# vqdang/hover_net

Measured on AMD Instinct MI355X. Metric: tiles/sec (270x270, batch 32) end-to-end incl. watershed, higher is better.
Workload: dtype fp32

## Files before the change

### hover_net_amd/csrc/hvn_api.hip

```cpp
#include <hip/hip_runtime.h>
#include <stdio.h>
#include <string.h>

#include <vector>

#include "../../include/hvn.h"
#include "hvn_kernels.h"

static thread_local char g_err[512] = "";

static int fail(int code, const char *fmt, const char *a = "", long b = 0)
{
    snprintf(g_err, sizeof(g_err), fmt, a, b);
    return code;
}

extern "C" {

int hvn_version(void) { return 104; }

#ifndef HVN_BUILD_ID
#define HVN_BUILD_ID "unstamped"
#endif
static const char hvn_build_tag[] = "hvn-build-id:" HVN_BUILD_ID;
// ... 141 lines not shown
        a.xsn = op->x.sn; a.xsy = op->x.sy; a.xsx = op->x.sx; a.K1 = op->x.c;
        a.x2 = (const float *)op->x2.base;
        a.x2sn = op->x2.sn; a.x2sy = op->x2.sy; a.x2sx = op->x2.sx;
        a.K1b = a.x2 ? op->x2.c : 0;
        a.stride2 = op->_rsv > 0 ? op->_rsv : 1;
        a.w1 = op->w;
        a.res = (const float *)op->res.base;
        a.rsn = op->res.sn; a.rsy = op->res.sy; a.rsx = op->res.sx;
        a.y = (float *)op->y.base;
        a.ysn = op->y.sn; a.ysy = op->y.sy; a.ysx = op->y.sx; a.C = op->cout;
        a.post_s = op->post_scale; a.post_b = op->post_shift;
        a.pre_s = op->pre_scale; a.pre_b = op->pre_shift;
        a.w2 = op->w2; a.bias2 = op->bias2; a.relu2 = 1;
        a.y2 = (float *)op->y2.base;
        a.y2sn = op->y2.sn; a.y2sy = op->y2.sy; a.y2sx = op->y2.sx; a.N2 = op->cout2;
        a.N = batch; a.Ho = op->y.h; a.Wo = op->y.w;
        a.M = (long)batch * a.Ho * a.Wo;
        a.bm = op->tile_n == 64 ? 64 : 128;
        const bool cx3 = op->act_dtype == 2 || op->act_dtype == 3;
        const bool cbf = op->act_dtype == 1;
        if (op->act_dtype != 0 && !cx3 && !cbf) return fail(HVN_E_ARG, "chain: act_dtype 0 (fp32), 1 (bf16) or 2 | 3 (fp32 with bf16x3 products)%s", "");
        if (cbf) {
            if (!a.x || !a.w1 || !a.y || !a.w2 || !a.y2) return fail(HVN_E_ARG, "chain: null pointer%s", "");
            if (op->kh != 1 || op->kw != 1 || op->stride != 1 || op->pad_t || op->pad_l || op->relu || op->bias)
                return fail(HVN_E_ARG, "chain: the first conv is a plain 1x1 (no bias / relu of its own)%s", "");
            if (!hvn_chain_bf16_supported(a.K1, a.K1b, a.C, a.N2) || op->y.c != a.C || op->y2.c != a.N2)
                return fail(HVN_E_ARG, "chain (bf16): needs input channels in slabs of 64 (64 or 128 in all), cout %% 256 == 0, cout2 in {64, 128} (cout2 = %s%ld)", "", a.N2);
            if (op->x.h != a.Ho || op->x.w != a.Wo || op->y2.h != a.Ho || op->y2.w != a.Wo ||
                (a.x2 && ((long)(a.Ho - 1) * a.stride2 >= op->x2.h || (long)(a.Wo - 1) * a.stride2 >= op->x2.w)))
                return fail(HVN_E_ARG, "chain: views do not cover the output grid%s", "");
            if (a.res && (a.rsn != a.ysn || a.rsy != a.ysy || a.rsx != a.ysx || op->res.c != a.C))
                return fail(HVN_E_ARG, "chain: the residual view must have the output's strides%s", "");
            if (!aligned16(a.x) || !aligned16(a.w1) || !aligned16(a.w2) || !aligned16(a.y) || !aligned16(a.y2) || (a.res && !aligned16(a.res)) ||
                (a.x2 && !aligned16(a.x2)) || ((a.xsn | a.xsy | a.xsx | a.ysn | a.ysy | a.ysx | a.y2sn | a.y2sy | a.y2sx | a.x2sn | a.x2sy | a.x2sx) & 7))
                return fail(HVN_E_ARG, "chain (bf16): views / weights not 16-byte aligned%s", "");
            if ((!a.pre_s != !a.pre_b) || (!a.post_s != !a.post_b) || (a.pre_s && (!aligned16(a.pre_s) || !aligned16(a.pre_b))) ||
                (a.post_s && (!aligned16(a.post_s) || !aligned16(a.post_b))) || (a.bias2 && !aligned16(a.bias2)))
                return fail(HVN_E_ARG, "chain: per-channel vectors must be 16-byte aligned and come in pairs%s", "");
            if (g_prof) prof_mark(s);
            const int rcb = hvn_launch_conv_chain_bf16(a, s);
            if (g_prof) prof_mark(s);
            if (rcb) return fail(rcb == -1 ? HVN_E_ARG : HVN_E_LAUNCH, "chain (bf16): launch failed (cout2=%s%ld)", "", a.N2);
            return 0;
        }
        if (!a.x || !a.w1 || !a.y || !a.w2 || !a.y2) return fail(HVN_E_ARG, "chain: null pointer%s", "");
        if (op->kh != 1 || op->kw != 1 || op->stride != 1 || op->pad_t || op->pad_l || op->relu || op->bias)
            return fail(HVN_E_ARG, "chain: the first conv is a plain 1x1 (no bias / relu of its own)%s", "");
        if (!hvn_chain_supported(a.C, a.N2) || op->y.c != a.C || op->y2.c != a.N2 || a.K1 % 32 || a.K1b % 32 || a.K1 + a.K1b < 64)
            return fail(HVN_E_ARG, "chain: needs cout %% 64 == 0, cout2 in {64, 128}, input channels in slabs of 32 (>= 64) (cout2 = %s%ld)", "", a.N2);
        if (op->x.h != a.Ho || op->x.w != a.Wo || op->y2.h != a.Ho || op->y2.w != a.Wo ||
            (a.x2 && ((long)(a.Ho - 1) * a.stride2 >= op->x2.h || (long)(a.Wo - 1) * a.stride2 >= op->x2.w)))
            return fail(HVN_E_ARG, "chain: views do not cover the output grid%s", "");
        if (a.res && (a.rsn != a.ysn || a.rsy != a.ysy || a.rsx != a.ysx || op->res.c != a.C))
            return fail(HVN_E_ARG, "chain: the residual view must have the output's strides%s", "");
        if (!aligned16(a.x) || !aligned16(a.w1) || !aligned16(a.w2) || !aligned16(a.y) || !aligned16(a.y2) || (a.res && !aligned16(a.res)) ||
            (a.x2 && !aligned16(a.x2)) || ((a.xsn | a.xsy | a.xsx | a.ysn | a.ysy | a.ysx | a.y2sn | a.y2sy | a.y2sx | a.x2sn | a.x2sy | a.x2sx) & 3))
            return fail(HVN_E_ARG, "chain: views / weights not 16-byte aligned%s", "");
        if ((!a.pre_s != !a.pre_b) || (!a.post_s != !a.post_b) || (a.pre_s && (!aligned16(a.pre_s) || !aligned16(a.pre_b))) ||
            (a.post_s && (!aligned16(a.post_s) || !aligned16(a.post_b))) || (a.bias2 && !aligned16(a.bias2)))
            return fail(HVN_E_ARG, "chain: per-channel vectors must be 16-byte aligned and come in pairs%s", "");
        if (g_prof) prof_mark(s);
        int rc;
        if (cx3 && op->tile_n == 1152)
            rc = hvn_launch_conv_chain_x3r(a, op->act_dtype == 3 ? 6 : 9, s);
        else
            rc = cx3 ? hvn_launch_conv_chain_x3(a, op->act_dtype == 3 ? 6 : 9, s) : hvn_launch_conv_chain(a, s);
        if (g_prof) prof_mark(s);
        if (rc) return fail(rc == -1 ? HVN_E_ARG : HVN_E_LAUNCH, "chain: launch failed (cout2=%s%ld)", "", a.N2);
        return 0;
    }
    case HVN_OP_WINO_IN:
    case HVN_OP_WINO_OUT: {
        WinoArgs a;
        const bool in = op->kind == HVN_OP_WINO_IN;
        a.x = (const float *)op->x.base;
        a.xsn = op->x.sn; a.xsy = op->x.sy; a.xsx = op->x.sx;
        a.y = (float *)op->y.base;
        a.ysn = op->y.sn; a.ysy = op->y.sy; a.ysx = op->y.sx;
        a.mat = op->w; a.bias = op->bias;
        a.N = batch; a.H = in ? op->x.h : op->y.h; a.W = in ? op->x.w : op->y.w; a.C = in ? op->x.c : op->y.c;
        a.ty = op->kh; a.tx = op->kw; a.pad = op->pad_t; a.relu = op->relu;
        a.accum = (!in && op->res.base != nullptr) ? 1 : 0;
        a.lo = nullptr; a.lsn = a.lsy = a.lsx = 0;
        if (in && op->res.base) {
            a.lo = (const float *)op->res.base;
            a.lsn = op->res.sn; a.lsy = op->res.sy; a.lsx = op->res.sx;
            if (op->res.h * 2 != op->x.h || op->res.w * 2 != op->x.w || op->res.c != op->x.c || !aligned16(a.lo) || ((a.lsn | a.lsy | a.lsx) & 3))
                return fail(HVN_E_ARG, "wino_in: the half-resolution input must be x.h/2 x x.w/2 x x.c and 16-byte aligned%s", "");
        }
        if (a.accum && op->res.base != op->y.base) return fail(HVN_E_ARG, "wino_out: res must alias y (accumulate in place)%s", "");
        const int n2 = in ? op->y.h : op->x.h;
        if (op->stride > 1 && op->_rsv > 1) {
            a.m = op->stride; a.r = op->_rsv;
        } else {
            a.m = n2 == 36 ? 2 : n2 == 64 ? 4 : n2 == 100 ? 6 : 0; a.r = 5;
        }
        if (!a.m || (a.m + a.r - 1) * (a.m + a.r - 1) != n2 || !((a.m == 2 && a.r == 5) || ((a.m == 4 || a.m == 6) && (a.r == 5 || a.r == 3))))
            return fail(HVN_E_ARG, "winograd transform: %s%ld transform positions do not match F(2,5) / F(4,5) / F(4,3) / F(6,3) / F(6,5)", "", (long)n2);
        if (!a.x || !a.y || !a.mat || a.ty <= 0 || a.tx <= 0 || (a.C & 3)) return fail(HVN_E_ARG, "winograd transform: bad descriptor%s", "");
        if (!aligned16(a.x) || !aligned16(a.y) || ((a.xsn | a.xsy | a.xsx | a.ysn | a.ysy | a.ysx) & 3))
            return fail(HVN_E_ARG, "winograd transform: views not 16-byte aligned%s", "");
        if (in && (op->y.w != a.ty * a.tx || op->y.c != a.C)) return fail(HVN_E_ARG, "wino_in: V must be [n*n][tiles][c]%s", "");
        if (!in && (op->x.w != a.ty * a.tx || op->y.h > a.m * a.ty || op->y.h <= a.m * (a.ty - 1) || op->y.w > a.m * a.tx ||
                    op->y.w <= a.m * (a.tx - 1) || op->x.c != a.C))
            return fail(HVN_E_ARG, "wino_out: M must be [n*n][tiles][cout] and the tiles must cover y%s", "");
        if (g_prof) prof_mark(s);
        int rc = in ? hvn_launch_wino_in(a, s) : hvn_launch_wino_out(a, s);
        if (g_prof) prof_mark(s);
        return rc;
    }
    case HVN_OP_UPADD: {
        UpAddArgs a;
        a.lo = (const float *)op->x.base;
        a.lsn = op->x.sn; a.lsy = op->x.sy; a.lsx = op->x.sx;
        a.skip = (const float *)op->res.base;
        a.ssn = op->res.sn; a.ssy = op->res.sy; a.ssx = op->res.sx;
        a.y = (float *)op->y.base;
        a.ysn = op->y.sn; a.ysy = op->y.sy; a.ysx = op->y.sx;
        a.N = batch; a.H = op->y.h; a.W = op->y.w; a.C = op->y.c; a.bf16 = op->act_dtype == 1;
        if (a.bf16 && ((a.lsx | a.lsy | a.lsn | a.ssx | a.ssy | a.ssn | a.ysx | a.ysy | a.ysn) & 7))
            return fail(HVN_E_ARG, "upadd(bf16): strides must be multiples of 8 elements%s", "");
        if (!a.lo || !a.skip || !a.y) return fail(HVN_E_ARG, "upadd: null pointer%s", "");
        if (op->x.h * 2 != a.H || op->x.w * 2 != a.W || op->res.h != a.H || op->res.w != a.W || op->x.c != a.C || op->res.c != a.C)
            return fail(HVN_E_ARG, "upadd: shape mismatch%s", "");
        if (!aligned16(a.lo) || !aligned16(a.skip) || !aligned16(a.y) || ((a.lsx | a.lsy | a.lsn | a.ssx | a.ssy | a.ssn | a.ysx | a.ysy | a.ysn) & 3))
            return fail(HVN_E_ARG, "upadd: views not 16-byte aligned%s", "");
        return hvn_launch_upadd(a, s);
    }
    case HVN_OP_HEAD: {
        HeadArgs a;
        a.x = (const float *)op->x.base;
        a.xsn = op->x.sn; a.xsy = op->x.sy; a.xsx = op->x.sx;
        a.w = op->w; a.bias = op->bias;
        a.y = (float *)op->y.base;
        a.N = batch; a.H = op->x.h; a.W = op->x.w; a.Cout = op->cout; a.in_bf16 = op->act_dtype == 1;
        if (a.in_bf16 && ((a.xsx | a.xsy | a.xsn) & 7)) return fail(HVN_E_ARG, "head(bf16): strides must be multiples of 8 elements%s", "");
        if (op->x.c != 64 || !a.w || !a.bias || !a.x || !a.y) return fail(HVN_E_ARG, "head: expects 64 input channels, weights and bias%s", "");
        if (!aligned16(a.x) || ((a.xsx | a.xsy | a.xsn) & 3)) return fail(HVN_E_ARG, "head: input view not 16-byte aligned%s", "");
        return hvn_launch_head(a, s);
    }
    case HVN_OP_PREDMAP: {
        PredMapArgs a;
        a.np = (const float *)op->x.base;
        a.hv = (const float *)op->res.base;
        a.tp = op->w;
        a.y = (float *)op->y.base;
        a.N = batch; a.H = op->y.h; a.W = op->y.w; a.nr_types = op->cout;
        if (!a.np || !a.hv || !a.y || (a.nr_types > 0 && !a.tp)) return fail(HVN_E_ARG, "predmap: null pointer%s", "");
        if (a.nr_types > 0 && !aligned16(a.y)) return fail(HVN_E_ARG, "predmap: output not 16-byte aligned%s", "");
        return hvn_launch_predmap(a, s);
    }
    default:
        return fail(HVN_E_ARG, "unknown op kind %s%ld", "", op->kind);
    }
}

}
int hvn_internal_run_one(const hvn_op *op, int batch, hipStream_t s) { return run_one(op, batch, s); }
extern "C" {

int hvn_run_op(const hvn_op *op, int batch, void *stream)
{
    if (!op || batch <= 0) return fail(HVN_E_ARG, "run_op: bad arguments%s", "");
    int rc = run_one(op, batch, (hipStream_t)stream);
    if (rc == -2) return fail(HVN_E_LAUNCH, "launch failed: %s", hipGetErrorString(hipGetLastError()));
    return rc;
// ... 102 lines not shown
```

### hover_net_amd/csrc/hvn_kernels.h

```cpp
#pragma once
#include <hip/hip_runtime.h>
#include <stdint.h>

#include <atomic>

static inline int hvn_max_lds_once(const void *kern, int bytes, std::atomic<unsigned long long> &done)
{
    int dev = 0;
    if (hipGetDevice(&dev) != hipSuccess) return -2;
    const unsigned long long bit = 1ull << (dev & 63);
    if (done.load(std::memory_order_acquire) & bit) return 0;
    if (hipFuncSetAttribute(kern, hipFuncAttributeMaxDynamicSharedMemorySize, bytes) != hipSuccess) return -2;
    done.fetch_or(bit, std::memory_order_release);
    return 0;
}

struct ConvArgs {
    const float *x;
    long xsn, xsy, xsx;
    int H, W, Cin;
    const float *w;
    const float *bias, *pre_s, *pre_b, *post_s, *post_b;
    const float *res;
    long rsn, rsy, rsx;
// ... 56 lines not shown
int hvn_launch_conv_chain_x3r(const ChainArgs &a, int terms, hipStream_t stream);
int hvn_launch_conv_bf16(const ConvArgs &a, int tile_n, hipStream_t stream);
int hvn_launch_conv_bf16g(const ConvArgs &a, int bm, hipStream_t stream);
int hvn_launch_conv_x3(const ConvArgs &a, int tile_n, int terms, hipStream_t stream);
int hvn_launch_conv_x3g(const ConvArgs &a, int bm, int terms, hipStream_t stream);
int hvn_conv_x3g_supported(const ConvArgs &a, int bm);
int hvn_launch_split_x3(const float *src, uint16_t *dst, long granules, hipStream_t stream);

struct Conv0Args {
    const void *img;
    long isn, isy, isx, isc;
    int is_f32;
    int H, W;
    const float *w;
    const float *bias;
    float *y;
    long ysn, ysy, ysx;
    int N, Ho, Wo, pad;
    int relu;
    int out_bf16;
};
int hvn_launch_conv0(const Conv0Args &a, hipStream_t stream);

struct UpAddArgs {
    const float *lo;
    long lsn, lsy, lsx;
    const float *skip;
    long ssn, ssy, ssx;
    float *y;
    long ysn, ysy, ysx;
    int N, H, W, C;
    int bf16;
};
int hvn_launch_upadd(const UpAddArgs &a, hipStream_t stream);

struct HeadArgs {
    const float *x;
    long xsn, xsy, xsx;
    const float *w;
    const float *bias;
    float *y;
    int N, H, W, Cout;
    int in_bf16;
};
int hvn_launch_head(const HeadArgs &a, hipStream_t stream);

int hvn_launch_extract_patches(const uint8_t *img, int H, int W, const int32_t *coords, int P, int win, int pad_t, int pad_l, uint8_t *out,
                               hipStream_t stream);

int hvn_launch_resize_window(const uint8_t *src, int src_h, int src_w, int64_t src_pitch, int src_y0, int src_x0, int full_h, int full_w,
                             const int32_t *xofs, const int16_t *xcoef, const int32_t *yofs, const int16_t *ycoef, int taps, uint8_t *dst,
                             int dst_h, int dst_w, hipStream_t stream);

size_t hvn_tissue_workspace_bytes(int h, int w);
int hvn_launch_tissue_gray_hist(const uint8_t *rgb, int h, int w, uint8_t *gray, uint32_t *hist256, hipStream_t stream);
int hvn_launch_tissue_mask(const uint8_t *gray, int h, int w, int threshold, int min_obj, int max_hole, int radius, uint8_t *mask,
                           uint8_t *tap_objects, uint8_t *tap_holes, void *workspace, hipStream_t stream);

int hvn_launch_viz_strip(const uint8_t *img, int n, int ih, int iw, const float *pred, int c, const int32_t *np_map, const float *hv_map,
                         const int32_t *tp_map, int h, int w, int nr_types, const int32_t *sel, int n_sel, const uint8_t *lut, uint8_t *out,
                         int n_blocks, hipStream_t stream);

struct PredMapArgs {
    const float *tp, *np, *hv;
    float *y;
    int N, H, W, nr_types;
};
int hvn_launch_predmap(const PredMapArgs &a, hipStream_t stream);

struct WinoArgs {
    const float *x;
    long xsn, xsy, xsx;
    float *y;
    long ysn, ysy, ysx;
    const float *mat;
    const float *bias;
    int N, H, W, C;
    int ty, tx, pad, relu;
    int m;
    int r;
    int accum;
    const float *lo;
    long lsn, lsy, lsx;
};
int hvn_launch_wino_in(const WinoArgs &a, hipStream_t stream);
int hvn_launch_wino_out(const WinoArgs &a, hipStream_t stream);

struct PackArgs {
    const float *src;
    float *dst;
    int cout, cin_g, groups, taps;
    int mode;
    int lead_pad;
    const float *gmat;
};
int hvn_launch_pack_w(const PackArgs &a, hipStream_t stream);
int hvn_launch_pack_w_multi(const PackArgs *tbl, const int *first_block, int n, long blocks, hipStream_t stream);

struct WgradArgs {
    const float *x;
    long xsn, xsy, xsx;
    int H, W, Cin;
    const float *dy;
    long dsn, dsy, dsx;
    int Ho, Wo, Cout;
    float *dw;
    int N, KH, KW, stride, pad_t, pad_l, groups, Cin_g;
    int tiles_m, tiles_n;
    unsigned rows_per_split;
    int nbatch;
    long xb, db, wb;
    int want_wgs;
    float *part;
    long part_stride, part_cap;
};
int hvn_launch_wgrad(const WgradArgs &a, hipStream_t stream);
long hvn_wgrad_split(const WgradArgs &a, long tiles, unsigned *rows_per_split);
long hvn_wgrad_part_floats(const WgradArgs &a, int x3);
int hvn_launch_reduce_parts(float *dst, const float *part, long elems, long nparts, long stride, hipStream_t stream);
int hvn_wgrad_x3_supported(const WgradArgs &a);
int hvn_launch_wgrad_x3(WgradArgs a, int terms, hipStream_t stream);
int hvn_launch_wino_dy(const struct WinoArgs &a, hipStream_t stream);
int hvn_launch_wino_dw(const float *du, float *dg, const float *gmat, int cout, int cin, hipStream_t stream);

#define HVN_BN_MAX_PARTS 256
struct BnArgs {
    const float *z;
    long zsn, zsy, zsx;
    const float *a;
    float *a_out;
    long asn, asy, asx;
    const float *da;
    long gsn, gsy, gsx;
    float *dz;
    long dsn, dsy, dsx;
    double *ws;
    float *save;
    float *coef;
    const float *gamma, *beta;
    float *dgamma, *dbeta, *running_mean, *running_var;
    int N, H, W, C, lq, nparts;
    float eps, momentum;
    int dz_store;
};
int hvn_launch_bn_forward(BnArgs a, hipStream_t stream);
int hvn_launch_bn_backward(BnArgs a, hipStream_t stream);

struct UpAddBwdArgs {
    const float *dy;
    long ysn, ysy, ysx;
    float *dlo;
    long lsn, lsy, lsx;
    float *dskip;
    long ssn, ssy, ssx;
    int N, H, W, C;
};
int hvn_launch_upadd_bwd(const UpAddBwdArgs &a, hipStream_t stream);

struct HeadBwdArgs {
    const float *x;
    long xsn, xsy, xsx;
    float *dx;
    long dsn, dsy, dsx;
    const float *dl;
    const float *w;
    float *dw, *db;
// ... 59 lines not shown
```

### hover_net_amd/csrc/hvn_net_ops.hip

```cpp
#include <hip/hip_runtime.h>
#include <stdlib.h>
#include <stdint.h>

#include "hvn_conv_common.h"

#define C0_T 16
#define C0_P (C0_T + 6)
template <typename T>
__global__ __launch_bounds__(256) void hvn_conv0(const Conv0Args p)
{
    __shared__ float patch[C0_P][C0_P * 3 + 2];
    const int tid = threadIdx.x;
    const int n = blockIdx.z;
    const int oy0 = blockIdx.y * C0_T, ox0 = blockIdx.x * C0_T;
    const T *img = (const T *)p.img + (long)n * p.isn;
    for (int i = tid; i < C0_P * C0_P * 3; i += 256) {
        const int py = i / (C0_P * 3), pr = i - py * (C0_P * 3);
        const int px = pr / 3, ch = pr - px * 3;
        const int iy = oy0 + py - p.pad, ix = ox0 + px - p.pad;
        float v = 0.f;
        if ((unsigned)iy < (unsigned)p.H && (unsigned)ix < (unsigned)p.W) v = (float)img[(long)iy * p.isy + (long)ix * p.isx + (long)ch * p.isc];
        patch[py][pr] = v;
    }
    __syncthreads();
// ... 247 lines not shown
        *(float4 *)(p.y + i * 4) = make_float4((float)best, prob, h, v);
    } else {
        float *y = p.y + i * 3;
        y[0] = prob;
        y[1] = h;
        y[2] = v;
    }
}

int hvn_launch_predmap(const PredMapArgs &a, hipStream_t stream)
{
    const long total = (long)a.N * a.H * a.W;
    hipLaunchKernelGGL(hvn_predmap, dim3((unsigned)((total + 255) / 256)), dim3(256), 0, stream, a, total);
    return hipGetLastError() == hipSuccess ? 0 : -2;
}

#ifndef HVN_WINO_XCD
#define HVN_WINO_XCD 1
#endif
template <int VW> struct WVec;
template <> struct WVec<4> { typedef float T __attribute__((ext_vector_type(4))); };
template <> struct WVec<2> { typedef float T __attribute__((ext_vector_type(2))); };
template <> struct WVec<1> { typedef float T __attribute__((ext_vector_type(1))); };

template <int MO, int R, int VW>
__global__ __launch_bounds__(256) void hvn_wino_in(const WinoArgs p, long total)
{
    constexpr int NW = MO + R - 1;
    typedef typename WVec<VW>::T VT;
    unsigned bid = blockIdx.x;
#if HVN_WINO_XCD
    {
        const unsigned per = gridDim.x >> 3;
        if (bid < per * 8) bid = (bid & 7) * per + (bid >> 3);
    }
#endif
    const long i = (long)bid * 256 + threadIdx.x;
    if (i >= total) return;
    const int cvn = p.C / VW;
    const int cv = (int)(i % cvn);
    long t = i / cvn;
    const int T1 = p.ty * p.tx;
    const int tile = (int)(t % T1);
    const int n = (int)(t / T1);
    const int tyi = tile / p.tx, txi = tile - tyi * p.tx;
    const int y0 = MO * tyi - p.pad, x0 = MO * txi - p.pad;
    float bt[NW * NW];
#pragma unroll
    for (int k = 0; k < NW * NW; ++k) bt[k] = p.mat[k];
    const float *src = p.x + (long)n * p.xsn + cv * VW;
    const float *lo = p.lo ? p.lo + (long)n * p.lsn + cv * VW : nullptr;
    VT tmp[NW][NW];
#pragma unroll
    for (int j = 0; j < NW; ++j) {
        VT d[NW];
#pragma unroll
        for (int r = 0; r < NW; ++r) {
            const int yy = y0 + r, xx = x0 + j;
            const bool in = (unsigned)yy < (unsigned)p.H && (unsigned)xx < (unsigned)p.W;
            VT v = in ? *(const VT *)(src + (long)yy * p.xsy + (long)xx * p.xsx) : (VT)(0.f);
            if (lo && in) v = *(const VT *)(lo + (long)(yy >> 1) * p.lsy + (long)(xx >> 1) * p.lsx) + v;
            d[r] = v;
        }
#pragma unroll
        for (int a = 0; a < NW; ++a) {
            VT s = (VT)(0.f);
#pragma unroll
            for (int r = 0; r < NW; ++r) s = __builtin_elementwise_fma((VT)(bt[a * NW + r]), d[r], s);
            tmp[a][j] = s;
        }
    }
    float *dst = p.y + (long)n * p.ysn + (long)tile * p.ysx + cv * VW;
#pragma unroll
    for (int a = 0; a < NW; ++a)
#pragma unroll
        for (int b = 0; b < NW; ++b) {
            VT s = (VT)(0.f);
#pragma unroll
            for (int j = 0; j < NW; ++j) s = __builtin_elementwise_fma((VT)(bt[b * NW + j]), tmp[a][j], s);
            *(VT *)(dst + (long)(a * NW + b) * p.ysy) = s;
        }
}

int hvn_launch_wino_in(const WinoArgs &a, hipStream_t stream)
{
    if (a.m == 2 && a.r == 5) {
        const long total = (long)a.N * a.ty * a.tx * (a.C / 4);
        hipLaunchKernelGGL((hvn_wino_in<2, 5, 4>), dim3((unsigned)((total + 255) / 256)), dim3(256), 0, stream, a, total);
    } else if (a.m == 4 && a.r == 3) {
        const long total = (long)a.N * a.ty * a.tx * (a.C / 4);
        hipLaunchKernelGGL((hvn_wino_in<4, 3, 4>), dim3((unsigned)((total + 255) / 256)), dim3(256), 0, stream, a, total);
    } else if (a.m == 4 && a.r == 5) {
        const long total = (long)a.N * a.ty * a.tx * (a.C / 2);
        hipLaunchKernelGGL((hvn_wino_in<4, 5, 2>), dim3((unsigned)((total + 255) / 256)), dim3(256), 0, stream, a, total);
    } else if (a.m == 6 && a.r == 3) {
        const long total = (long)a.N * a.ty * a.tx * (a.C / 2);
        hipLaunchKernelGGL((hvn_wino_in<6, 3, 2>), dim3((unsigned)((total + 255) / 256)), dim3(256), 0, stream, a, total);
    } else if (a.m == 6 && a.r == 5) {
        const long total = (long)a.N * a.ty * a.tx * a.C;
        hipLaunchKernelGGL((hvn_wino_in<6, 5, 1>), dim3((unsigned)((total + 255) / 256)), dim3(256), 0, stream, a, total);
    } else
        return -1;
    return hipGetLastError() == hipSuccess ? 0 : -2;
}

template <int MO, int R, int VW>
__global__ __launch_bounds__(256) void hvn_wino_out(const WinoArgs p, long total)
{
    constexpr int NW = MO + R - 1;
    typedef typename WVec<VW>::T VT;
    const long i = (long)blockIdx.x * 256 + threadIdx.x;
    if (i >= total) return;
    const int c4n = p.C / VW;
    const int c4 = (int)(i % c4n);
    long t = i / c4n;
    const int T1 = p.ty * p.tx;
    const int tile = (int)(t % T1);
    const int n = (int)(t / T1);
    const int tyi = tile / p.tx, txi = tile - tyi * p.tx;
    float at[MO * NW];
#pragma unroll
    for (int k = 0; k < MO * NW; ++k) at[k] = p.mat[k];
    const float *src = p.x + (long)n * p.xsn + (long)tile * p.xsx + c4 * VW;
    VT tmp[MO][NW];
#pragma unroll
    for (int b = 0; b < NW; ++b) {
        VT m[NW];
#pragma unroll
        for (int a = 0; a < NW; ++a) m[a] = *(const VT *)(src + (long)(a * NW + b) * p.xsy);
#pragma unroll
        for (int q = 0; q < MO; ++q) {
            VT s = (VT)(0.f);
#pragma unroll
            for (int a = 0; a < NW; ++a) s = __builtin_elementwise_fma((VT)(at[q * NW + a]), m[a], s);
            tmp[q][b] = s;
        }
    }
    VT bias = (VT)(0.f);
    if (p.bias) bias = *(const VT *)(p.bias + c4 * VW);
    const float lo = p.relu ? 0.f : -__builtin_inff();
    float *dst = p.y + (long)n * p.ysn + c4 * VW;
#pragma unroll
    for (int q = 0; q < MO; ++q)
#pragma unroll
        for (int r = 0; r < MO; ++r) {
            VT s = bias;
#pragma unroll
            for (int b = 0; b < NW; ++b) s = __builtin_elementwise_fma((VT)(at[r * NW + b]), tmp[q][b], s);
            s = __builtin_elementwise_max(s, (VT)(lo));
            const int oy = MO * tyi + q, ox = MO * txi + r;
            if (oy < p.H && ox < p.W) {
                VT *d = (VT *)(dst + (long)oy * p.ysy + (long)ox * p.ysx);
                *d = p.accum ? *d + s : s;
            }
        }
}

int hvn_launch_wino_out(const WinoArgs &a, hipStream_t stream)
{
    if (a.m == 2 && a.r == 5) {
        const long total = (long)a.N * a.ty * a.tx * (a.C / 4);
        hipLaunchKernelGGL((hvn_wino_out<2, 5, 4>), dim3((unsigned)((total + 255) / 256)), dim3(256), 0, stream, a, total);
    } else if (a.m == 4 && a.r == 3) {
        const long total = (long)a.N * a.ty * a.tx * (a.C / 4);
        hipLaunchKernelGGL((hvn_wino_out<4, 3, 4>), dim3((unsigned)((total + 255) / 256)), dim3(256), 0, stream, a, total);
    } else if (a.m == 4 && a.r == 5) {
        const long total = (long)a.N * a.ty * a.tx * (a.C / 2);
        hipLaunchKernelGGL((hvn_wino_out<4, 5, 2>), dim3((unsigned)((total + 255) / 256)), dim3(256), 0, stream, a, total);
// ... 46 lines not shown
```

### hover_net_amd/engine.py

```python
import ctypes

import numpy as np
import torch

from . import lib as L
from . import plan as PL
from . import tune as T
from .tune import X3G_128, X3G_256, X3R


def _view_struct(v, base_ptr, sn, itemsize=4):
    b = v.buf
    sx = b.c
    sy = b.w * b.c
    s = L.hvn_view()
    s.base = base_ptr + (v.y0 * sy + v.x0 * sx + v.c0) * itemsize
    s.sn, s.sy, s.sx = sn, sy, sx
    s.h, s.w, s.c, s.sc = v.h, v.w, v.c, 1
    return s


_STREAM_POOL = {}


# ... 5 lines not shown


def to_bf16_bits(a):
    u = np.ascontiguousarray(a, np.float32).view(np.uint32)
    return ((u + (((u >> 16) & 1) + 0x7FFF)) >> 16).astype(np.uint16)


def repack_conv_bf16(w32):
    cp, s32, taps, _ = w32.shape
    if s32 % 2:
        w32 = np.concatenate([w32, np.zeros((cp, 1, taps, 32), np.float32)], 1)
        s32 += 1
    w = w32.reshape(cp, s32 // 2, 2, taps, 32).transpose(0, 1, 3, 2, 4).reshape(cp, s32 // 2, taps, 64)
    return to_bf16_bits(w)


def split_bf16x3(w32):
    w = np.ascontiguousarray(w32, np.float32)

    def bf(a):
        bits = to_bf16_bits(a)
        return bits, (bits.astype(np.uint32) << 16).view(np.float32)

    h, hf = bf(w)
    r = w - hf
    m, mf = bf(r)
    l, _ = bf(r - mf)
    return h, m, l


def pack_conv_x3(w32):
    lead = w32.shape[:-3]
    kt = w32.shape[-3] * w32.shape[-2]
    planes = split_bf16x3(w32.reshape(lead + (kt, 32)))
    return np.stack(planes, axis=-2)


def pack_conv_x3_device(w32, device):
    w = torch.from_numpy(np.ascontiguousarray(w32, np.float32).reshape(-1, 32)).to(device)
    h = w.to(torch.bfloat16)
    r = w - h.float()
    m = r.to(torch.bfloat16)
    l = (r - m.float()).to(torch.bfloat16)
    return torch.stack((h, m, l), dim=1).view(torch.int16).reshape(-1)


class Engine:
    def __init__(self, plan, max_batch=32, device="cuda", n_split=None, dtype="fp32", n_lanes=None):
        L.require_gpu()
        assert dtype in ("fp32", "bf16")
        self.dtype = dtype
        self.isz = 4 if dtype == "fp32" else 2
        if dtype == "bf16" and any(op.kind in (PL.OP_WINO_IN, PL.OP_WINO_OUT) for op in plan.ops):
            raise ValueError("the bf16 path runs direct convolutions: build the plan with winograd=0")
        self.plan = plan
        self.max_batch = int(max_batch)
        self.device = torch.device(device)
        import os
        dflt = ("2", "2") if dtype == "fp32" else ("1", "0")
        self.n_split = int(os.environ.get("HVN_SPLIT", dflt[0])) if n_split is None else int(n_split)
        self.n_lane_streams = int(os.environ.get("HVN_LANES", dflt[1])) if n_lanes is None else int(n_lanes)
        self.split_decoder = os.environ.get("HVN_SPLIT_DECODER", "0") != "0"
        self._streams = None
        self._stream_off = 0
        self._upload_params()
        self.arena = torch.empty((self.max_batch, plan.arena_per_sample), dtype=torch.float32 if dtype == "fp32" else torch.int16,
                                 device=self.device)
        self.logits = {br: torch.empty((self.max_batch, b.c, b.h, b.w), dtype=torch.float32, device=self.device)
                       for br, b in plan.logits.items()}
        self.pred_map = None
        if plan.pred_map is not None:
            pm = plan.pred_map
            self.pred_map = torch.empty((self.max_batch, pm.h, pm.w, pm.c), dtype=torch.float32, device=self.device)
        self.ops = (L.hvn_op * len(plan.ops))()
        self._bind()
        self._sub_ops = {}
        tile_file = T.knob("HVN_TILE_FILE")
        if tile_file and dtype == "fp32":
            import json
            tiles = json.load(open(tile_file))
            if len(tiles) != len(self.ops):
                raise ValueError("HVN_TILE_FILE holds %d entries for a plan of %d ops" % (len(tiles), len(self.ops)))
            for o, tn in zip(self.ops, tiles):
                if tn in T.candidates(o):
                    o.tile_n = tn
        elif T.tile_select() == "auto" and not (dtype == "fp32" and T.knob("HVN_FORCE_TILE_N")):
            self.autotune_tiles()
        if T.tile_select() == "auto" and T.knob("HVN_STREAM_SELECT") != "0":
            self.autotune_streams()

    def _upload_params(self):
        arrays, offs, total = [], {}, 0

        def put(key, a):
            nonlocal total
            if a is None:
                return
            a = np.ascontiguousarray(a, np.float32).ravel()
            offs[key] = total
            arrays.append((total, a))
            total += (a.size + 63) // 64 * 64

        w16, off16, tot16 = [], {}, 0
        for i, op in enumerate(self.plan.ops):
            if self.dtype == "bf16" and op.kind in (PL.OP_CONV, PL.OP_CHAIN):
                wb = repack_conv_bf16(op.w).ravel()
                off16[i] = tot16
                w16.append((tot16, wb))
                tot16 += (wb.size + 127) // 128 * 128
                if op.kind == PL.OP_CHAIN:
                    wb2 = repack_conv_bf16(op.extra["w2"]).ravel()
                    off16[(i, "w2")] = tot16
                    w16.append((tot16, wb2))
                    tot16 += (wb2.size + 127) // 128 * 128
            elif self.dtype == "fp32" and op.kind in (PL.OP_CONV, PL.OP_CHAIN) and op.extra.get("x3"):
                off16[i] = tot16
                w16.append((tot16, op.w, True))
                tot16 += (3 * op.w.size + 127) // 128 * 128
                if op.kind == PL.OP_CHAIN:
                    off16[(i, "w2")] = tot16
                    w16.append((tot16, op.extra["w2"], True))
                    tot16 += (3 * op.extra["w2"].size + 127) // 128 * 128
            else:
                put((i, "w"), op.w)
            put((i, "bias"), op.bias)
            if not (op.kind == PL.OP_CHAIN and (self.dtype == "bf16" or op.extra.get("x3"))):
                put((i, "w2"), op.extra.get("w2"))
            put((i, "bias2"), op.extra.get("bias2"))
            if op.pre is not None:
                put((i, "pre_s"), op.pre[0])
                put((i, "pre_b"), op.pre[1])
            if op.post is not None:
                put((i, "post_s"), op.post[0])
                put((i, "post_b"), op.post[1])
        host = np.zeros(max(total, 64), np.float32)
        for off, a in arrays:
            host[off:off + a.size] = a
        self.params = torch.from_numpy(host).to(self.device)
        self._poff = offs
        self._poff16 = off16
        self.params16 = None
        if tot16:
            if any(len(e) == 3 for e in w16):
                self.params16 = torch.zeros(tot16, dtype=torch.int16, device=self.device)
                for off, w32, _ in w16:
                    pl = pack_conv_x3_device(w32, self.device)
                    self.params16[off:off + pl.numel()] = pl
            else:
                h16 = np.zeros(tot16, np.uint16)
                for off, a in w16:
                    h16[off:off + a.size] = a
                self.params16 = torch.from_numpy(h16.view(np.int16)).to(self.device)

    def _pptr(self, i, name):
        off = self._poff.get((i, name))
        return None if off is None else self.params.data_ptr() + 4 * off

    def _bind(self):
        P = self.plan
        abase = self.arena.data_ptr()
        sn = P.arena_per_sample
        for i, op in enumerate(P.ops):
            o = self.ops[i]
            o.act_dtype = 1 if self.dtype == "bf16" else 0
            o.kind, o.kh, o.kw, o.stride = op.kind, op.kh, op.kw, op.stride
            o.pad_t, o.pad_l, o.relu, o.cout, o.tile_n, o.x_dtype = op.pad_t, op.pad_l, op.relu, op.cout, op.tile_n, 0
            if op.kind == PL.OP_CONV and self.dtype == "fp32":
                o.tile_n = T.pick_tile_n(op, self.max_batch)
            o.groups = int(op.extra.get("groups", 1))
            o._rsv = int(op.extra.get("stride2", 1))
            o.nbatch = int(op.extra.get("nbatch", 1))
            for bi, bs in enumerate(op.extra.get("batch_strides", (0, 0, 0))):
                o.batch_stride[bi] = int(bs)
            if op.kind in (PL.OP_WINO_IN, PL.OP_WINO_OUT):
                o.kh, o.kw = op.extra["tiles"]
                o.stride, o._rsv = op.extra["m"], op.extra.get("r", 5)
            if op.kind == PL.OP_PREDMAP:
                o.x.base = self.logits["np"].data_ptr()
                o.res.base = self.logits["hv"].data_ptr()
                o.w = self.logits["tp"].data_ptr() if "tp" in self.logits else None
                o.cout = P.nr_types or 0
                o.y.base = self.pred_map.data_ptr()
                o.y.h, o.y.w, o.y.c = P.pred_map.h, P.pred_map.w, P.pred_map.c
                continue
            if op.kind == PL.OP_CHAIN:
                o.cout2 = int(op.extra["cout2"])
                o.w2, o.bias2 = self._pptr(i, "w2"), self._pptr(i, "bias2")
                if self.dtype == "bf16":
                    o.w2 = self.params16.data_ptr() + 2 * self._poff16[(i, "w2")]
                elif op.extra.get("x3"):
                    o.w2 = self.params16.data_ptr() + 2 * self._poff16[(i, "w2")]
                    o.act_dtype = 2 if int(op.extra["x3"]) == 9 else 3
                    o.tile_n = 128
            for fld, v in (("x", op.x), ("res", op.res), ("y", op.y), ("x2", op.extra.get("x2")), ("y2", op.extra.get("y2"))):
                if v is None:
                    continue
                if v.buf.offset >= 0:
                    setattr(o, fld, _view_struct(v, abase + self.isz * v.buf.offset, sn, self.isz))
            if op.kind == PL.OP_CONV0:
                o.x.h, o.x.w, o.x.c = op.x.h, op.x.w, 3
            if op.kind == PL.OP_HEAD:
                br = op.y.buf.name.split(".")[1]
                o.y.base = self.logits[br].data_ptr()
                o.y.h, o.y.w, o.y.c = op.y.h, op.y.w, op.y.c
            o.w = self._pptr(i, "w") if i not in self._poff16 else self.params16.data_ptr() + 2 * self._poff16[i]
            if i in self._poff16 and self.dtype == "bf16":
                o.groups = 1
            if self.dtype == "fp32" and op.kind == PL.OP_CONV and op.extra.get("x3"):
                o.act_dtype = 2 if int(op.extra["x3"]) == 9 else 3
                if o.nbatch > 1:
                    o.batch_stride[1] = int(op.w.shape[-4]) * int(op.w.shape[-3]) * int(op.w.shape[-2]) * 96
            o.bias = self._pptr(i, "bias")
            o.pre_scale, o.pre_shift = self._pptr(i, "pre_s"), self._pptr(i, "pre_b")
            o.post_scale, o.post_shift = self._pptr(i, "post_s"), self._pptr(i, "post_b")

    def autotune_streams(self):
        split = self.n_split if (self.n_split > 1 and self.max_batch >= 2 * self.n_split) else 1
        need = (split - 1) + split * self.n_lane_streams
        if need == 0 or self.plan.ops[0].kind != PL.OP_CONV0 or not getattr(self.plan, "geo", None):
            return
        g = int(self.plan.geo.get("inp", 0))
        if g <= 0:
            return
        imgs = torch.zeros((self.max_batch, g, g, 3), dtype=torch.uint8, device=self.device)

        def measure(off):
            self._stream_off, self._streams = off, None
            return T.time_launch(lambda: self.run(imgs), runs=2)

        key = (str(self.device), "streams", split, self.n_lane_streams, self.dtype)
        self._stream_off, self._streams = T.choose(T.CACHE, key, (0, 1, 2, 3), measure, margin=1.0)[0], None

    def autotune_tiles(self):
        run_op = L.lib().hvn_run_op
        stream = L.stream_ptr(self.device)
        osz = ctypes.sizeof(L.hvn_op)
        base = ctypes.addressof(self.ops)
        lanes = getattr(self.plan, "lanes", None)
        enc_end = lanes[0][2] if (lanes and lanes[0][0] == "main" and len(lanes) > 1) else 0
        split = self.n_split if (self.n_split > 1 and self.max_batch >= 2 * self.n_split) else 1
        sub_n = -(-self.max_batch // split) if T.knob("HVN_TUNE_SUB") != "0" else self.max_batch
        for i, o in enumerate(self.ops):
            cands = T.candidates(o)
            if not cands:
                continue
            nb = sub_n if (i < enc_end or self.split_decoder) else self.max_batch
            family = "infer-bf16" if o.act_dtype == 1 else "infer-conv" if o.kind == PL.OP_CONV else "infer-chain-x3" if o.act_dtype else "infer-chain"

            def measure(tn):
                o.tile_n = tn
                return T.time_launch(lambda: L.check(run_op(base + i * osz, nb, stream), "hvn_run_op (autotune)"))

            o.tile_n = T.pick(T.CACHE, T.launch_key(self.device, family, o, nb), cands, measure, forced=T.forced_form(o))
        torch.cuda.synchronize(self.device)

    def _set_input(self, imgs):
        o = self.ops[0]
        assert self.plan.ops[0].kind == PL.OP_CONV0
        n = imgs.shape[0]
        if n > self.max_batch:
            raise ValueError("batch %d exceeds the engine's max_batch %d" % (n, self.max_batch))
        g = self.plan.geo["inp"]
        if imgs.dtype == torch.uint8:
            if tuple(imgs.shape[1:]) != (g, g, 3):
                raise ValueError("expected uint8 [N,%d,%d,3] patches, got %s" % (g, g, tuple(imgs.shape)))
            imgs = imgs.contiguous()
            o.x_dtype = 0
            o.x.sn, o.x.sy, o.x.sx, o.x.sc = g * g * 3, g * 3, 3, 1
        elif imgs.dtype == torch.float32:
            if tuple(imgs.shape[1:]) != (3, g, g):
                raise ValueError("expected float32 [N,3,%d,%d] images, got %s" % (g, g, tuple(imgs.shape)))
            imgs = imgs.contiguous()
            o.x_dtype = 1
            o.x.sn, o.x.sy, o.x.sx, o.x.sc = 3 * g * g, g, 1, g * g
        else:
            raise TypeError("images must be uint8 NHWC or float32 NCHW, got %s" % imgs.dtype)
        if imgs.device != self.device:
            imgs = imgs.to(self.device, non_blocking=True)
        o.x.base = imgs.data_ptr()
        return imgs, n

    def run_raw(self, n):
        L.call("hvn_run_plan", ctypes.addressof(self.ops), len(self.ops), n, L.stream_ptr(self.device))

    def _shifted_ops(self, first):
        key = first
        if key not in self._sub_ops:
            ops = (L.hvn_op * len(self.ops))()
            ctypes.memmove(ops, self.ops, ctypes.sizeof(self.ops))
            for i, op in enumerate(self.plan.ops):
                o = ops[i]
                for fld in ("x", "res", "y", "x2", "y2"):
                    v = getattr(o, fld)
                    if v.base:
                        if op.kind == PL.OP_HEAD and fld == "y":
                            v.base += 4 * first * op.y.c * op.y.h * op.y.w
                        elif op.kind == PL.OP_PREDMAP:
                            c = {"x": 2, "res": 2, "y": self.plan.pred_map.c}[fld]
                            v.base += 4 * first * c * self.plan.pred_map.h * self.plan.pred_map.w
                        elif op.kind == PL.OP_CONV0 and fld == "x":
                            pass
                        else:
                            v.base += self.isz * first * v.sn
                if op.kind == PL.OP_PREDMAP and o.w:
                    o.w += 4 * first * (self.plan.nr_types or 0) * self.plan.pred_map.h * self.plan.pred_map.w
            self._sub_ops[key] = ops
        return self._sub_ops[key]

    def _launch(self, ops, n_ops, cnt, stream, lane_streams, start=0):
        run_plan = L.lib().hvn_run_plan
        base = ctypes.addressof(ops)
        osz = ctypes.sizeof(L.hvn_op)
        sp = L.stream_ptr(stream=stream)
        lanes = getattr(self.plan, "lanes", None)
        if not lanes or not lane_streams or n_ops != len(self.ops):
            L.check(run_plan(base + start * osz, n_ops - start, cnt, sp), "hvn_run_plan")
            return
        branch_i = 0
        pending = []
        for lane, lo, hi in lanes:
            lo = max(lo, start)
            if lo >= hi:
                continue
            if lane == "main":
                for ev in pending:
                    stream.wait_event(ev)
                pending = []
                L.check(run_plan(base + lo * osz, hi - lo, cnt, sp), "hvn_run_plan")
            else:
                st = stream if branch_i == 0 else lane_streams[(branch_i - 1) % len(lane_streams)]
                if st is not stream:
                    fork = torch.cuda.Event()
                    fork.record(stream)
                    st.wait_event(fork)
                L.check(run_plan(base + lo * osz, hi - lo, cnt, sp if st is stream else L.stream_ptr(stream=st)), "hvn_run_plan")
                if st is not stream:
# ... 71 lines not shown
```

### hover_net_amd/tune.py

```python
import math
import os

import torch

from . import lib as L
from .plan import OP_CHAIN, OP_CONV, _tile_n

KNOBS = {
    "HVN_TILE_SELECT": ("auto", "auto: forms picked by time at engine build | model: inference CONV tiles by pick_tile_n's rounds model, nothing timed | 0: the plan's static tiles"),
    "HVN_TUNE_REPS": ("", "timings per candidate after the warm-up launch (default 3; 2 for the weight-gradient stream pass)"),
    "HVN_TUNE_SUB": ("1", "0: a split inference engine times its encoder launches at the full batch instead of the sub-batch"),
    "HVN_FORCE_TILE_N": ("", "64 | 128: that column tile for every re-tileable fp32 inference CONV, nothing timed"),
    "HVN_WG_SLOTS_64": ("768", "rounds model: resident 128x64 workgroups on the chip"),
    "HVN_NARROW_COST": ("0.45", "rounds model: time of a round of 128x64 tiles relative to a round of 128x128 tiles"),
    "HVN_X3G": ("1", "LDS-DMA forms of the bf16x3 CONV: 0 none | 896 | 640 that form only | 1 both"),
    "HVN_X3G_FORCE": ("", "896 | 640: that bf16x3 LDS-DMA form wherever it is a candidate, nothing timed"),
    "HVN_BF16G": ("1", "0: no LDS-DMA forms of the bf16 CONV"),
    "HVN_BF16G_FORCE": ("", "896 | 640: that bf16 LDS-DMA form wherever it is a candidate, nothing timed"),
    "HVN_CHAIN_X3R": ("1", "register-resident form of the bf16x3 CHAIN: 0 never | force wherever it is a candidate | 1 by time"),
    "HVN_STREAM_SELECT": ("1", "0: the inference launch schedule keeps rotation 0 of the stream pool"),
    "HVN_TILE_SHARE": ("1", "0: data-parallel ranks keep their own measured launch shapes (no broadcast from rank 0)"),
    "HVN_TILE_FILE": ("", "path of a JSON list of per-op tile_n codes an fp32 inference engine binds instead of timing"),
}

MARGIN = 0.985
X3G_256, X3G_128 = 128 + 0x300, 128 + 0x200
X3R = 128 + 0x400
T256X64 = 64 + 0x100
OPTIONAL = (X3G_256, X3G_128, X3R)
WGRAD_TARGETS = (1536, 1024, 768, 512, 384)
WG_SLOTS = 512

CACHE = {}


def knob(name):
    return os.environ.get(name, KNOBS[name][0])


def tile_select():
    v = knob("HVN_TILE_SELECT")
    if v not in ("auto", "model", "0"):
        raise ValueError("HVN_TILE_SELECT=%r: auto, model or 0" % v)
    return v


def time_launch(launch, reps=3, runs=1):
    reps = max(1, int(knob("HVN_TUNE_REPS") or reps))
    e0, e1 = torch.cuda.Event(enable_timing=True), torch.cuda.Event(enable_timing=True)
    best = float("inf")
    for r in range(reps + 1):
        e0.record()
        for _ in range(runs):
            launch()
        e1.record()
        e1.synchronize()
        if r:
            best = min(best, e0.elapsed_time(e1) / runs)
    return best


def choose(cache, key, candidates, measure, margin=MARGIN, optional=OPTIONAL):
    key = tuple(key) + (tuple(candidates),)
    if key not in cache:
        t = {}
        for c in candidates:
            try:
                t[c] = measure(c)
            except L.HvnError:
                if c not in optional:
                    raise
                t[c] = float("inf")
        base = candidates[0]
        best = min(candidates[1:], key=t.get)
        cache[key] = (best if t[best] < margin * t[base] else base, t[base], t[best], t)
    return cache[key]


def forced_form(o):
    if o.kind == OP_CHAIN:
        return X3R if knob("HVN_CHAIN_X3R") == "force" else None
    v = knob("HVN_BF16G_FORCE" if o.act_dtype == 1 else "HVN_X3G_FORCE")
    return int(v) if v else None


def pick(cache, key, candidates, measure, forced=None, optional=OPTIONAL, **kw):
    if forced in optional and forced in candidates[1:]:
        try:
            measure(forced)
            return forced
        except L.HvnError:
            return candidates[0]
    return choose(cache, key, candidates, measure, optional=optional, **kw)[0]


def entries(family, device=None):
    return [(k, v) for k, v in CACHE.items() if k[1] == family and (device is None or k[0] == str(device))]


def launch_key(device, family, o, batch):
    return (str(device), family, int(batch), o.kh, o.kw, o.stride, o.pad_t, o.x.c, o.cout, o.cout2, o.y.h, o.y.w, o.x.h, o.x.w, bool(o.res.base),
            bool(o.pre_scale), bool(o.post_scale), int(o.nbatch), int(o.x2.c) if o.x2.base else 0, int(o.act_dtype), int(o.groups))


def x3g_forms_for(o):
    want = knob("HVN_X3G")
    if want == "0" or o.cout < 128 or o.groups > 1:
        return ()
    forms = []
    for code, bm, na in ((X3G_256, 256, 3), (X3G_128, 128, 2)):
        if want not in ("1", str(code)):
            continue
        if o.pre_scale and bm == 256 and na * bm * 128 + 2 * 3 * 128 * 64 + 2 * o.x.c * 4 > 160 * 1024:
            continue
        forms.append(code)
    return tuple(forms)


def candidates(o):
    x3, bf16 = o.act_dtype in (2, 3), o.act_dtype == 1
    if o.kind == OP_CHAIN:
        if x3:
            if knob("HVN_CHAIN_X3R") == "0" or o.x.c != 64 or (o.x2.base and (o.x2.c != 64 or o.res.base or o.cout2 != 64)):
                return ()
            return (128, X3R)
        return () if bf16 else (128, 64)
    if o.kind != OP_CONV or o.groups > 1:
        return ()
    static = _tile_n(o.cout)
    if bf16:
        if static != 128 or o.pre_scale or o.nbatch > 1 or knob("HVN_BF16G") == "0":
            return ()
        return (128, X3G_256, X3G_128)
    if static == 128:
        return (128, 64) + (x3g_forms_for(o) if x3 else ())
    if static == 64 and not x3 and not o.x2.base:
        return (64, T256X64)
    return ()


def pick_tile_n(op, batch):
    if op.tile_n != 128 or tile_select() == "0":
        return op.tile_n
    force = knob("HVN_FORCE_TILE_N")
    if force:
        return int(force)
    slots64 = int(knob("HVN_WG_SLOTS_64"))
    cost64 = float(knob("HVN_NARROW_COST"))
    m_tiles = math.ceil(batch * op.y.h * op.y.w / 128.0)
    nb = int(op.extra.get("nbatch", 1))
    wide = math.ceil(m_tiles * math.ceil(op.cout / 128.0) * nb / WG_SLOTS)
    narrow = math.ceil(m_tiles * math.ceil(op.cout / 64.0) * nb / slots64) * cost64
    return 64 if narrow < wide else 128
```

Baseline: 748.8.

## Add strip-cooperative LDS Winograd input transform kernel with autotuned selection

Adds a new Winograd input-transform kernel in which a 256-thread block stages a row strip of tiles and a 32-channel slab in LDS. It then runs the column and row transforms from shared memory, so overlapping tile halos are loaded once instead of per thread. It also fuses the upsampled half-resolution residual add into the staging. The form is exposed as tile_n=1 and chosen by autotune timing against the existing per-thread kernel, by default only for WINO_IN ops that carry a low-res input. This adds LDS use and two block barriers per strip.

```diff
diff --git a/hover_net_amd/csrc/hvn_api.hip b/hover_net_amd/csrc/hvn_api.hip
--- a/hover_net_amd/csrc/hvn_api.hip
+++ b/hover_net_amd/csrc/hvn_api.hip
@@ -247,6 +247,8 @@
         a.ty = op->kh; a.tx = op->kw; a.pad = op->pad_t; a.relu = op->relu;
         a.accum = (!in && op->res.base != nullptr) ? 1 : 0;
         a.lo = nullptr; a.lsn = a.lsy = a.lsx = 0;
+        a.form = in ? op->tile_n : 0;
+        if (a.form != 0 && a.form != 1) return fail(HVN_E_ARG, "wino_in: tile_n must be 0 (per-thread kernel) or 1 (strip kernel)%s", "");
         if (in && op->res.base) {
             a.lo = (const float *)op->res.base;
             a.lsn = op->res.sn; a.lsy = op->res.sy; a.lsx = op->res.sx;
diff --git a/hover_net_amd/csrc/hvn_kernels.h b/hover_net_amd/csrc/hvn_kernels.h
--- a/hover_net_amd/csrc/hvn_kernels.h
+++ b/hover_net_amd/csrc/hvn_kernels.h
@@ -162,6 +162,7 @@
     int accum;
     const float *lo;
     long lsn, lsy, lsx;
+    int form;
 };
 int hvn_launch_wino_in(const WinoArgs &a, hipStream_t stream);
 int hvn_launch_wino_out(const WinoArgs &a, hipStream_t stream);
diff --git a/hover_net_amd/csrc/hvn_net_ops.hip b/hover_net_amd/csrc/hvn_net_ops.hip
--- a/hover_net_amd/csrc/hvn_net_ops.hip
+++ b/hover_net_amd/csrc/hvn_net_ops.hip
@@ -353,8 +353,170 @@
         }
 }
 
+#ifndef HVN_WS_SLAB
+#define HVN_WS_SLAB 32
+#endif
+#ifndef HVN_WS_COLS
+#define HVN_WS_COLS(nw) ((nw) == 10 ? 24 : (nw) == 8 ? 32 : 40)
+#endif
+
+template <int MO, int R>
+__global__ __launch_bounds__(256) void hvn_wino_in_strip(const WinoArgs p, int run, int runs, int slabs)
+{
+    constexpr int NW = MO + R - 1, S4 = HVN_WS_SLAB / 4, PITCH = HVN_WS_COLS(NW) + 1;
+    constexpr int UB = 4, UP = 8;
+    typedef typename WVec<4>::T VT;
+    static_assert(!(NW & 1) && !(MO & 1) && !(S4 & (S4 - 1)), "2 x 2 blocks tile the strip; the float4 index is a mask");
+    __shared__ VT sm[NW * PITCH * S4];
+    unsigned bid = blockIdx.x;
+#if HVN_WINO_XCD
+    {
+        const unsigned per = gridDim.x >> 3;
+        if (bid < per * 8) bid = (bid & 7) * per + (bid >> 3);
+    }
+#endif
+    const int tid = threadIdx.x;
+    const int slab = (int)(bid % (unsigned)slabs);
+    unsigned t = bid / (unsigned)slabs;
+    const int rn = (int)(t % (unsigned)runs);
+    t /= (unsigned)runs;
+    const int tyi = (int)(t % (unsigned)p.ty);
+    const int n = (int)(t / (unsigned)p.ty);
+    const int tx0 = rn * run;
+    const int nt = min(run, p.tx - tx0);
+    if (nt <= 0) return;
+    const int cols = nt * MO + R - 1;
+    const int y0 = MO * tyi - p.pad, x0 = MO * tx0 - p.pad;
+    const int c0 = slab * HVN_WS_SLAB;
+    const int nc4 = min(S4, (p.C - c0) >> 2);
+    const float *src = p.x + (long)n * p.xsn + c0;
+    const float *lo = p.lo ? p.lo + (long)n * p.lsn + c0 : nullptr;
+    if (lo && !((p.pad | p.H | p.W) & 1)) {
+        const int bc = cols >> 1, tot = (NW / 2) * bc * S4;
+        for (int e0 = tid; e0 < tot; e0 += 256 * UB) {
+            VT v[UB][4];
+            int at[UB];
+#pragma unroll
+            for (int u = 0; u < UB; ++u) {
+                const int e = e0 + u * 256;
+                const int c4 = e & (S4 - 1), b = e / S4, br = b / bc, bj = b - br * bc;
+                const int yy = y0 + 2 * br, xx = x0 + 2 * bj;
+                const bool in = e < tot && c4 < nc4 && (unsigned)yy < (unsigned)p.H && (unsigned)xx < (unsigned)p.W;
+                const long off = in ? (long)yy * p.xsy + (long)xx * p.xsx + c4 * 4 : 0;
+                const long offl = in ? (long)(yy >> 1) * p.lsy + (long)(xx >> 1) * p.lsx + c4 * 4 : 0;
+                const VT l = *(const VT *)(lo + offl);
+                const VT z = (VT)(0.f);
+                v[u][0] = in ? l + *(const VT *)(src + off) : z;
+                v[u][1] = in ? l + *(const VT *)(src + off + p.xsx) : z;
+                v[u][2] = in ? l + *(const VT *)(src + off + p.xsy) : z;
+                v[u][3] = in ? l + *(const VT *)(src + off + p.xsy + p.xsx) : z;
+                at[u] = e < tot ? ((2 * br) * PITCH + 2 * bj) * S4 + c4 : -1;
+            }
+#pragma unroll
+            for (int u = 0; u < UB; ++u)
+                if (at[u] >= 0) {
+                    sm[at[u]] = v[u][0];
+                    sm[at[u] + S4] = v[u][1];
+                    sm[at[u] + PITCH * S4] = v[u][2];
+                    sm[at[u] + PITCH * S4 + S4] = v[u][3];
+                }
+        }
+    } else {
+        const int tot = NW * cols * S4;
+        for (int e0 = tid; e0 < tot; e0 += 256 * UP) {
+            VT v[UP];
+            int at[UP];
+#pragma unroll
+            for (int u = 0; u < UP; ++u) {
+                const int e = e0 + u * 256;
+                const int c4 = e & (S4 - 1), px = e / S4, r = px / cols, j = px - r * cols;
+                const int yy = y0 + r, xx = x0 + j;
+                const bool in = e < tot && c4 < nc4 && (unsigned)yy < (unsigned)p.H && (unsigned)xx < (unsigned)p.W;
+                const long off = in ? (long)yy * p.xsy + (long)xx * p.xsx + c4 * 4 : 0;
+                VT x = *(const VT *)(src + off);
+                if (lo) x = *(const VT *)(lo + (in ? (long)(yy >> 1) * p.lsy + (long)(xx >> 1) * p.lsx + c4 * 4 : 0)) + x;
+                v[u] = in ? x : (VT)(0.f);
+                at[u] = e < tot ? (r * PITCH + j) * S4 + c4 : -1;
+            }
+#pragma unroll
+            for (int u = 0; u < UP; ++u)
+                if (at[u] >= 0) sm[at[u]] = v[u];
+        }
+    }
+    __syncthreads();
+    const float *__restrict__ mat = p.mat;
+    for (int e = tid; e < cols * S4; e += 256) {
+        VT *col = sm + e;
+        VT d[NW];
+#pragma unroll
+        for (int r = 0; r < NW; ++r) d[r] = col[r * PITCH * S4];
+        float cur[NW], nxt[NW];
+#pragma unroll
+        for (int r = 0; r < NW; ++r) cur[r] = mat[r];
+#pragma unroll 1
+        for (int a = 0; a < NW; ++a) {
+            const int an = a + 1 < NW ? a + 1 : a;
+#pragma unroll
+            for (int r = 0; r < NW; ++r) nxt[r] = mat[an * NW + r];
+            VT s = (VT)(0.f);
+#pragma unroll
+            for (int r = 0; r < NW; ++r) s = __builtin_elementwise_fma((VT)(cur[r]), d[r], s);
+            col[a * PITCH * S4] = s;
+#pragma unroll
+            for (int r = 0; r < NW; ++r) cur[r] = nxt[r];
+        }
+    }
+    __syncthreads();
+    float *dst0 = p.y + (long)n * p.ysn + (long)(tyi * p.tx + tx0) * p.ysx + c0;
+    for (int e = tid; e < nt * NW * S4; e += 256) {
+        const int c4 = e & (S4 - 1), q = e / S4, tl = q / NW, a = q - tl * NW;
+        if (c4 >= nc4) continue;
+        const VT *row = sm + (a * PITCH + tl * MO) * S4 + c4;
+        VT tm[NW];
+#pragma unroll
+        for (int j = 0; j < NW; ++j) tm[j] = row[j * S4];
+        float *dst = dst0 + (long)tl * p.ysx + c4 * 4 + (long)(a * NW) * p.ysy;
+        float cur[NW], nxt[NW];
+#pragma unroll
+        for (int j = 0; j < NW; ++j) cur[j] = mat[j];
+#pragma unroll 1
+        for (int b = 0; b < NW; ++b) {
+            const int bn = b + 1 < NW ? b + 1 : b;
+#pragma unroll
+            for (int j = 0; j < NW; ++j) nxt[j] = mat[bn * NW + j];
+            VT s = (VT)(0.f);
+#pragma unroll
+            for (int j = 0; j < NW; ++j) s = __builtin_elementwise_fma((VT)(cur[j]), tm[j], s);
+            *(VT *)(dst + (long)b * p.ysy) = s;
+#pragma unroll
+            for (int j = 0; j < NW; ++j) cur[j] = nxt[j];
+        }
+    }
+}
+
+template <int MO, int R>
+static int hvn_wino_in_strip_launch(const WinoArgs &a, hipStream_t stream)
+{
+    constexpr int RUN_MAX = (HVN_WS_COLS(MO + R - 1) - (R - 1)) / MO;
+    const int runs = (a.tx + RUN_MAX - 1) / RUN_MAX;
+    const int run = (a.tx + runs - 1) / runs;
+    const int slabs = (a.C + HVN_WS_SLAB - 1) / HVN_WS_SLAB;
+    const long grid = (long)a.N * slabs * a.ty * runs;
+    if (grid <= 0 || grid > 0x7fffffffL) return -1;
+    hipLaunchKernelGGL((hvn_wino_in_strip<MO, R>), dim3((unsigned)grid), dim3(256), 0, stream, a, run, runs, slabs);
+    return hipGetLastError() == hipSuccess ? 0 : -2;
+}
+
 int hvn_launch_wino_in(const WinoArgs &a, hipStream_t stream)
 {
+    if (a.form == 1) {
+        if (a.m == 2 && a.r == 5) return hvn_wino_in_strip_launch<2, 5>(a, stream);
+        if (a.m == 4 && a.r == 3) return hvn_wino_in_strip_launch<4, 3>(a, stream);
+        if (a.m == 4 && a.r == 5) return hvn_wino_in_strip_launch<4, 5>(a, stream);
+        if (a.m == 6 && a.r == 3) return hvn_wino_in_strip_launch<6, 3>(a, stream);
+        if (a.m == 6 && a.r == 5) return hvn_wino_in_strip_launch<6, 5>(a, stream);
+        return -1;
+    }
     if (a.m == 2 && a.r == 5) {
         const long total = (long)a.N * a.ty * a.tx * (a.C / 4);
         hipLaunchKernelGGL((hvn_wino_in<2, 5, 4>), dim3((unsigned)((total + 255) / 256)), dim3(256), 0, stream, a, total);
diff --git a/hover_net_amd/engine.py b/hover_net_amd/engine.py
--- a/hover_net_amd/engine.py
+++ b/hover_net_amd/engine.py
@@ -111,7 +111,7 @@
             if len(tiles) != len(self.ops):
                 raise ValueError("HVN_TILE_FILE holds %d entries for a plan of %d ops" % (len(tiles), len(self.ops)))
             for o, tn in zip(self.ops, tiles):
-                if tn in T.candidates(o):
+                if tn in (T.candidates(o) or T.wino_in_forms(o)):
                     o.tile_n = tn
         elif T.tile_select() == "auto" and not (dtype == "fp32" and T.knob("HVN_FORCE_TILE_N")):
             self.autotune_tiles()
@@ -270,17 +270,18 @@
         split = self.n_split if (self.n_split > 1 and self.max_batch >= 2 * self.n_split) else 1
         sub_n = -(-self.max_batch // split) if T.knob("HVN_TUNE_SUB") != "0" else self.max_batch
         for i, o in enumerate(self.ops):
-            cands = T.candidates(o)
+            cands = T.candidates(o) or T.wino_in_forms(o)
             if not cands:
                 continue
             nb = sub_n if (i < enc_end or self.split_decoder) else self.max_batch
-            family = "infer-bf16" if o.act_dtype == 1 else "infer-conv" if o.kind == PL.OP_CONV else "infer-chain-x3" if o.act_dtype else "infer-chain"
+            family = "infer-wino-in" if o.kind == PL.OP_WINO_IN else "infer-bf16" if o.act_dtype == 1 else "infer-conv" if o.kind == PL.OP_CONV else "infer-chain-x3" if o.act_dtype else "infer-chain"
 
             def measure(tn):
                 o.tile_n = tn
                 return T.time_launch(lambda: L.check(run_op(base + i * osz, nb, stream), "hvn_run_op (autotune)"))
 
-            o.tile_n = T.pick(T.CACHE, T.launch_key(self.device, family, o, nb), cands, measure, forced=T.forced_form(o))
+            o.tile_n = T.pick(T.CACHE, T.launch_key(self.device, family, o, nb), cands, measure, forced=T.forced_form(o),
+                              optional=T.OPTIONAL + (T.WINO_STRIP,))
         torch.cuda.synchronize(self.device)
 
     def _set_input(self, imgs):
diff --git a/hover_net_amd/tune.py b/hover_net_amd/tune.py
--- a/hover_net_amd/tune.py
+++ b/hover_net_amd/tune.py
@@ -4,7 +4,7 @@
 import torch
 
 from . import lib as L
-from .plan import OP_CHAIN, OP_CONV, _tile_n
+from .plan import OP_CHAIN, OP_CONV, OP_WINO_IN, _tile_n
 
 KNOBS = {
     "HVN_TILE_SELECT": ("auto", "auto: forms picked by time at engine build | model: inference CONV tiles by pick_tile_n's rounds model, nothing timed | 0: the plan's static tiles"),
@@ -18,6 +18,7 @@
     "HVN_BF16G": ("1", "0: no LDS-DMA forms of the bf16 CONV"),
     "HVN_BF16G_FORCE": ("", "896 | 640: that bf16 LDS-DMA form wherever it is a candidate, nothing timed"),
     "HVN_CHAIN_X3R": ("1", "register-resident form of the bf16x3 CHAIN: 0 never | force wherever it is a candidate | 1 by time"),
+    "HVN_WINO_IN_STRIP": ("1", "strip-cooperative form of the inference WINO_IN: 0 never | force everywhere, nothing timed | 1 by time"),
     "HVN_STREAM_SELECT": ("1", "0: the inference launch schedule keeps rotation 0 of the stream pool"),
     "HVN_TILE_SHARE": ("1", "0: data-parallel ranks keep their own measured launch shapes (no broadcast from rank 0)"),
     "HVN_TILE_FILE": ("", "path of a JSON list of per-op tile_n codes an fp32 inference engine binds instead of timing"),
@@ -27,6 +28,7 @@
 X3G_256, X3G_128 = 128 + 0x300, 128 + 0x200
 X3R = 128 + 0x400
 T256X64 = 64 + 0x100
+WINO_STRIP = 1
 OPTIONAL = (X3G_256, X3G_128, X3R)
 WGRAD_TARGETS = (1536, 1024, 768, 512, 384)
 WG_SLOTS = 512
@@ -80,6 +82,8 @@
 def forced_form(o):
     if o.kind == OP_CHAIN:
         return X3R if knob("HVN_CHAIN_X3R") == "force" else None
+    if o.kind == OP_WINO_IN:
+        return WINO_STRIP if knob("HVN_WINO_IN_STRIP") == "force" else None
     v = knob("HVN_BF16G_FORCE" if o.act_dtype == 1 else "HVN_X3G_FORCE")
     return int(v) if v else None
 
@@ -139,6 +143,13 @@
     return ()
 
 
+def wino_in_forms(o):
+    want = knob("HVN_WINO_IN_STRIP")
+    if o.kind != OP_WINO_IN or o.act_dtype != 0 or want == "0" or not (o.res.base or want == "force"):
+        return ()
+    return (0, WINO_STRIP)
+
+
 def pick_tile_n(op, batch):
     if op.tile_n != 128 or tile_select() == "0":
         return op.tile_n
```

Measured after the change: 747.4 (median of 2 runs). No clear change (-0.2%).
